# jacobhinkle/lagomorph

Measured on AMD Instinct MI355X. Metric: LDDMM step voxels/sec (3D, 128^3), higher is better.
Workload: dtype f32; 1 GPU; lddmm.expmap, 10 Euler steps, global batch 32 x 3x128^3 fp32 sharded 32 per GPU (BASELINE configs[3]); value counts voxels x Euler steps; shooting from the identity, the first Euler step is evaluated in closed form (-dt sharp(m0): the bits EPDiff_step returns); the product's default path: each rank's shoot runs as 2 sub-batches on HIP streams of their own (lddmm.EXPMAP_STREAMS, bit-identical); streams=2, global_batch=32, per_gpu_batch=32, euler_steps=10

## Files before the change

### lagomorph_amd/csrc/fused.hip

```cpp
#include <algorithm>
#include <type_traits>
#include <stdlib.h>

#include "common.hpp"
#include "stencil_tile.hpp"
#include "gather_window.hpp"

namespace lago {

template <typename R, int DIM>
__global__ __launch_bounds__(kBlock) void compose_kernel(R *__restrict__ out, const R *__restrict__ u,
                                                         const R *__restrict__ v, double ds, double dt, Geom g) {
    const Vox vx = locate(g);
    if (!vx.valid) return;
    const size_t nv = g.nvox;
    const R *un = u + (size_t)vx.n * DIM * nv + vx.s;
    const R *vn = v + (size_t)vx.n * DIM * nv;
    R *on = out + (size_t)vx.n * DIM * nv + vx.s;
    const R dsr = (R)ds, dtr = (R)dt;
    R uv[DIM];
#pragma unroll
    for (int d = 0; d < DIM; ++d) uv[d] = un[(size_t)d * nv];
    if (DIM == 3) {
        Lerp3<R> L;
// ... 78 lines not shown
    const int lz = threadIdx.x & 31, ly = (threadIdx.x >> 5) & (GW::TY - 1), lxb = threadIdx.x / (32 * GW::TY);
    const int j = tl.y0 + ly, k = tl.z0 + lz;

    GWOrigin o;
    {
        const int cxi = min(tl.x0 + GW::TX / 2, g.nx - 1), cyi = min(tl.y0 + GW::TY / 2, g.ny - 1),
                  czi = min(tl.z0 + GW::TZ / 2, g.nz - 1);
        const uint32_t cs = ((uint32_t)cxi * (uint32_t)g.ny + (uint32_t)cyi) * (uint32_t)g.nz + (uint32_t)czi;
        o = gw_origin(tl, g, lg_floor(sample_pos_t<float, UNIT>(cxi, ds, un[cs])),
                      lg_floor(sample_pos_t<float, UNIT>(cyi, ds, un[nv + cs])),
                      lg_floor(sample_pos_t<float, UNIT>(czi, ds, un[2 * nv + cs])));
    }
    GWLoader<NT> ld;
    ld.plan(o, g);
    ld.issue(vn, plane, gwin);

    const bool row_ok = j < g.ny && k < g.nz;
    const uint32_t off0 = (((uint32_t)(tl.x0 + lxb) * (uint32_t)g.ny + (uint32_t)j) * (uint32_t)g.nz + (uint32_t)k) * 4u;
    const uint32_t estep = (uint32_t)XS * (uint32_t)g.ny * (uint32_t)g.nz * 4u;
    auto voff = [&](int e) { return row_ok && tl.x0 + lxb + XS * e < g.nx ? off0 + (uint32_t)e * estep : GW::kOutside; };
    GWLerp L[U];
    uint32_t outm = 0;
    float uu[3][U];
    {
#pragma unroll
        for (int e = 0; e < U; ++e) {
#pragma unroll
            for (int d = 0; d < 3; ++d)
                uu[d][e] = __builtin_bit_cast(float, __builtin_amdgcn_raw_buffer_load_b32(make_rsrc(un + (size_t)d * nv, plane), voff(e), 0, LAGO_COMPOSE_AUX_LD));
        }
#pragma unroll
        for (int e = 0; e < U; ++e) {
            const int i = tl.x0 + lxb + XS * e;
            const bool in = L[e].setup(sample_pos_t<float, UNIT>(i, ds, uu[0][e]), sample_pos_t<float, UNIT>(j, ds, uu[1][e]),
                                       sample_pos_t<float, UNIT>(k, ds, uu[2][e]), g, o);
            outm |= (in | (voff(e) == GW::kOutside)) ? 0u : 1u << e;
            __builtin_amdgcn_sched_barrier(0);
        }
    }
    auto channels = [&](auto stray) {
        constexpr bool STRAY = decltype(stray)::value;
#pragma unroll
        for (int c = 0; c < 3; ++c) {
            if (c > 0) {
                asm volatile("s_waitcnt vmcnt(0)" ::: "memory");
                __syncthreads();
            }
            const BufRsrc ro = make_rsrc(on + (size_t)c * nv, plane);
#pragma unroll
            for (int e = 0; e < U; ++e) {
                float val = L[e].value(gwin);
                if constexpr (STRAY) {
                    const bool mine = outm & (1u << e);
                    if (__builtin_amdgcn_ballot_w64(mine) != 0) {
                        if (mine) {
                            const int i = tl.x0 + lxb + XS * e;
                            Lerp3<float, false> P;
                            P.setup(sample_pos_t<float, UNIT>(i, ds, uu[0][e]), sample_pos_t<float, UNIT>(j, ds, uu[1][e]),
                                    sample_pos_t<float, UNIT>(k, ds, uu[2][e]), g.nx, g.ny, g.nz);
                            val = P.value(vn + (size_t)c * nv);
                        }
                    }
                }
                const float a = dsr * uu[c][e];
                const float b = dtr * val;
                __builtin_amdgcn_raw_buffer_store_b32(__builtin_bit_cast(uint32_t, a + b), ro, voff(e), 0, LAGO_COMPOSE_AUX_ST);
            }
            if (c < 2) {
                __syncthreads();
                ld.issue(vn + (size_t)(c + 1) * nv, plane, gwin);
            }
        }
    };
    asm volatile("s_waitcnt vmcnt(0)" ::: "memory");
    if (__syncthreads_or(outm != 0))
        channels(std::true_type{});
    else
        channels(std::false_type{});
}

template __global__ void compose3_window_kernel<GW::NT, 8, true>(float *, const float *, const float *, double, double, Geom, GWGrid);
template __global__ void compose3_window_kernel<GW::NT, 8, false>(float *, const float *, const float *, double, double, Geom, GWGrid);

std::atomic<int> g_gather_window{1};
std::atomic<int> g_tile_cube{1};

static size_t padded_smem(size_t smem) {
#ifdef LAGO_PROFILING
    static const size_t pad = [] {
        const char *e = getenv("LAGO_EXP_GATHER_PAD");
        return e ? (size_t)strtoul(e, nullptr, 10) : (size_t)0;
    }();
    if (pad > smem) smem = pad;
#endif
    return smem;
}

template <typename R>
static int compose_window_launch(R *out, const R *u, const R *v, double ds, double dt, const Geom &g, int64_t nn,
                                 hipStream_t s) {
    if constexpr (sizeof(R) == 4) {
        GWGrid w;
        if (!make_gwgrid(w, g, nn) || ((uintptr_t)v & 15u)) return kNotTaken;
        constexpr int NT = GW::NT, U = 8;
        const hipError_t e = with_flags([&](auto UNIT) {
            return launch(compose3_window_kernel<NT, U, UNIT()>, dim3(w.total), dim3(NT), padded_smem(GW::lds_bytes<NT>()), s,
                          out, u, v, ds, dt, g, w);
        }, unit_dt<R>(ds));
        if (e != hipSuccess) return fail_hip(e, "compose");
        note_path(LP_GATHER_WINDOW);
        return LAGO_OK;
    }
    return kNotTaken;
}

template <typename R>
static int compose_impl(R *out, const R *u, const R *v, double ds, double dt, int dim, int64_t nn, int64_t nx,
                        int64_t ny, int64_t nz, void *stream) {
    if (dim != 2 && dim != 3) return fail_invalid("Only two- and three-dimensional interpolation is supported");
    Geom g;
    if (!make_geom(g, dim, nn, nx, ny, nz)) return fail_invalid("compose: bad extent");
    if (g.nblocks == 0) return LAGO_OK;
    if (!out || !u || !v) return fail_invalid("compose: null pointer");
    hipStream_t s = (hipStream_t)stream;
    constexpr int U = 2;
    if (dim == 3 && g_interp_vec && g_gather_window && g.nvox >= 32768u) {
        const int rc = compose_window_launch(out, u, v, ds, dt, g, nn, s);
        if (rc != kNotTaken) return rc != LAGO_OK ? rc : finish_launch(s, "compose");
    }
    uint32_t nbx_u, nb;
    if (dim == 3 && g_interp_vec && slab_grid(g, nn, U, nbx_u, nb)) {
        with_flags([&](auto UNIT) {
            hipLaunchKernelGGL((compose3_unroll_kernel<R, U, UNIT()>), dim3(nb), dim3(kBlock), 0, s, out, u, v, ds, dt, g,
                               nbx_u, nb);
        }, unit_dt<R>(ds));
        note_path(LP_VECTOR_GATHER);
        return finish_launch(s, "compose");
    }
    with_dim(dim, [&](auto DIM) {
        hipLaunchKernelGGL((compose_kernel<R, DIM()>), dim3(g.nblocks), dim3(kBlock), 0, s, out, u, v, ds, dt, g);
    });
    return finish_launch(s, "compose");
}


template <typename R, int DIM>
__device__ __forceinline__ R jac_row_dot(int c, const R (&fp)[DIM], const R (&fm)[DIM], const R (&w)[DIM]) {
    R gq[DIM];
#pragma unroll
    for (int d = 0; d < DIM; ++d) {
        gq[d] = (R)0.5f * (fp[d] - fm[d]);
        if (c == d) gq[d] = gq[d] + (R)1.0;
    }
    const R sacc = lg_fma(gq[0], w[0], gq[1] * w[1]);
    return DIM == 3 ? lg_fma(gq[DIM - 1], w[DIM - 1], sacc) : sacc;
}

template <typename R, int DIM>
__global__ __launch_bounds__(kBlock) void ad_star_kernel(R *__restrict__ out, R *__restrict__ mphi,
                                                         const R *__restrict__ phi, const R *__restrict__ m, Geom g) {
    const Vox vx = locate(g);
    if (!vx.valid) return;
    const size_t nv = g.nvox;
    const R *pn = phi + (size_t)vx.n * DIM * nv + vx.s;
    const R *mn = m + (size_t)vx.n * DIM * nv;
    R *on = out + (size_t)vx.n * DIM * nv + vx.s;
    R pv[DIM], wv[DIM];
#pragma unroll
    for (int d = 0; d < DIM; ++d) pv[d] = pn[(size_t)d * nv];
    int plus[DIM], minus[DIM];
    if (DIM == 3) {
        Lerp3<R> L;
        L.setup(sample_pos<R>(vx.i, 1.0, pv[0]), sample_pos<R>(vx.j, 1.0, pv[1]), sample_pos<R>(vx.k, 1.0, pv[2]),
                g.nx, g.ny, g.nz);
#pragma unroll
        for (int d = 0; d < 3; ++d) wv[d] = L.value(mn + (size_t)d * nv);
        const int P[3] = {vx.i, vx.j, vx.k}, Ln[3] = {g.nx, g.ny, g.nz}, St[3] = {g.ny * g.nz, g.nz, 1};
#pragma unroll
        for (int d = 0; d < 3; ++d) {
            plus[d] = P[d] + 1 < Ln[d] ? St[d] : 0;
            minus[d] = P[d] > 0 ? -St[d] : 0;
        }
    } else {
        Lerp2<R> L;
        L.setup(sample_pos<R>(vx.j, 1.0, pv[0]), sample_pos<R>(vx.k, 1.0, pv[1]), g.ny, g.nz);
#pragma unroll
// ... 202 lines not shown
template <typename R>
static int ad_star_impl(R *out, R *mphi, const R *phi, const R *m, int dim, int64_t nn, int64_t nx, int64_t ny,
                        int64_t nz, void *stream) {
    if (dim != 2 && dim != 3) return fail_invalid("Only two- and three-dimensional fields are supported");
    Geom g;
    if (!make_geom(g, dim, nn, nx, ny, nz)) return fail_invalid("ad_star: bad extent");
    if (g.nblocks == 0) return LAGO_OK;
    if (!out || !phi || !m) return fail_invalid("ad_star: null pointer");
    if (out == phi || out == m || (mphi && (mphi == phi || mphi == m || mphi == out)))
        return fail_invalid("ad_star: outputs may not alias an input or each other");
    if (thin(dim, nx, ny, nz))
        return fail_invalid("Jacobian times vectorfield not implemented for 'thin' dimensions");
    hipStream_t s = (hipStream_t)stream;
    constexpr int U = 2;
    if (dim == 3 && g_interp_vec && g_stencil_tile && g.nvox >= 4096u) {
        const int rc = ad_star_tile_launch<R>(out, mphi, phi, m, g, nn, s);
        if (rc != kNotTaken) return rc != LAGO_OK ? rc : finish_launch(s, "ad_star");
    }
    uint32_t nbx_u, nb;
    if (dim == 3 && g_interp_vec && slab_grid(g, nn, U, nbx_u, nb)) {
        hipLaunchKernelGGL((ad_star3_unroll_kernel<R, U>), dim3(nb), dim3(kBlock), 0, s, out, mphi, phi, m, g, nbx_u, nb);
        note_path(LP_VECTOR_GATHER);
        return finish_launch(s, "ad_star");
    }
    with_dim(dim, [&](auto DIM) {
        hipLaunchKernelGGL((ad_star_kernel<R, DIM()>), dim3(g.nblocks), dim3(kBlock), 0, s, out, mphi, phi, m, g);
    });
    return finish_launch(s, "ad_star");
}

template <typename R, int K, int VEC>
__global__ __launch_bounds__(256) void lincomb_kernel(R *out, const R *x0, const R *x1, const R *x2, const R *x3, R c0,
                                                      R c1, R c2, R c3, size_t nvec, int rev) {
    struct alignas(sizeof(R) * VEC) V { R e[VEC]; };
    const size_t stride = (size_t)gridDim.x * blockDim.x;
    for (size_t j = (size_t)blockIdx.x * blockDim.x + threadIdx.x; j < nvec; j += stride) {
        const size_t i = rev ? nvec - 1 - j : j;
        const V a = reinterpret_cast<const V *>(x0)[i];
        V b = a, c = a, d = a, r;
        if (K > 1) b = reinterpret_cast<const V *>(x1)[i];
        if (K > 2) c = reinterpret_cast<const V *>(x2)[i];
        if (K > 3) d = reinterpret_cast<const V *>(x3)[i];
#pragma unroll
        for (int e = 0; e < VEC; ++e) {
            R acc = c0 * a.e[e];
            if (K > 1) acc = lg_fma(c1, b.e[e], acc);
            if (K > 2) acc = lg_fma(c2, c.e[e], acc);
            if (K > 3) acc = lg_fma(c3, d.e[e], acc);
            r.e[e] = acc;
        }
        reinterpret_cast<V *>(out)[i] = r;
    }
}

template <typename R>
int lincomb_impl(R *out, int k, const R *x0, const R *x1, const R *x2, const R *x3, double c0, double c1, double c2,
                 double c3, int64_t n, void *stream) {
    if (k < 1 || k > 4 || n < 0) return fail_invalid("lincomb: 1 to 4 terms");
    if (n == 0) return LAGO_OK;
    hipStream_t s = (hipStream_t)stream;
    constexpr int VEC = 16 / sizeof(R);
    auto aligned = [](const void *p) { return p == nullptr || (reinterpret_cast<uintptr_t>(p) & 15) == 0; };
    const bool vec = n % VEC == 0 && aligned(out) && aligned(x0) && aligned(k > 1 ? x1 : nullptr) &&
                     aligned(k > 2 ? x2 : nullptr) && aligned(k > 3 ? x3 : nullptr);
    const size_t nvec = vec ? (size_t)n / VEC : (size_t)n;
    const uint32_t grid = (uint32_t)std::min<size_t>((nvec + 255) / 256, (size_t)256 * 32);
    const int rev = next_direction();
    with_flags([&](auto WIDE) {
        constexpr int V = WIDE() ? VEC : 1;
        with_int<1, 2, 3, 4>(k, [&](auto K) {
            hipLaunchKernelGGL((lincomb_kernel<R, K(), V>), dim3(grid), dim3(256), 0, s, out, x0, x1, x2, x3, (R)c0, (R)c1,
                               (R)c2, (R)c3, nvec, rev);
        });
    }, vec);
    return finish_launch(s, "lincomb");
}

}

namespace lago {
void tune_fused(int stencil_tile, int gather_window) {
    g_stencil_tile = stencil_tile ? 1 : 0;
    g_tile_cube = stencil_tile == 3 ? 0 : 1;
    g_gather_window = gather_window ? 1 : 0;
}
}

extern "C" {
int lago_lincomb_f32(float *out, int k, const float *x0, const float *x1, const float *x2, const float *x3, double c0,
                     double c1, double c2, double c3, int64_t n, void *stream) {
    return lago::lincomb_impl<float>(out, k, x0, x1, x2, x3, c0, c1, c2, c3, n, stream);
}
int lago_lincomb_f64(double *out, int k, const double *x0, const double *x1, const double *x2, const double *x3,
                     double c0, double c1, double c2, double c3, int64_t n, void *stream) {
    return lago::lincomb_impl<double>(out, k, x0, x1, x2, x3, c0, c1, c2, c3, n, stream);
}
int lago_compose_f32(float *out, const float *u, const float *v, double ds, double dt, int dim, int64_t nn,
                     int64_t nx, int64_t ny, int64_t nz, void *stream) {
    return lago::compose_impl<float>(out, u, v, ds, dt, dim, nn, nx, ny, nz, stream);
}
int lago_compose_f64(double *out, const double *u, const double *v, double ds, double dt, int dim, int64_t nn,
                     int64_t nx, int64_t ny, int64_t nz, void *stream) {
    return lago::compose_impl<double>(out, u, v, ds, dt, dim, nn, nx, ny, nz, stream);
}
int lago_Ad_star_f32(float *out, float *mphi, const float *phiinv, const float *m, int dim, int64_t nn, int64_t nx,
                     int64_t ny, int64_t nz, void *stream) {
    return lago::ad_star_impl<float>(out, mphi, phiinv, m, dim, nn, nx, ny, nz, stream);
}
int lago_Ad_star_f64(double *out, double *mphi, const double *phiinv, const double *m, int dim, int64_t nn, int64_t nx,
                     int64_t ny, int64_t nz, void *stream) {
    return lago::ad_star_impl<double>(out, mphi, phiinv, m, dim, nn, nx, ny, nz, stream);
}
}
```

### lagomorph_amd/csrc/gather_window.hpp

```cpp
#pragma once
#include "common.hpp"

namespace lago {

struct GW {
#ifndef LAGO_GW_TY
#define LAGO_GW_TY 16
#endif
    static constexpr int TX = 8, TY = LAGO_GW_TY, TZ = 32, H = 2, HZ = 4;
    static constexpr int NT = 32 * TY;
    static constexpr int WX = TX + 1 + 2 * H, WY = TY + 1 + 2 * H, WZC = 11, WZ = 4 * WZC;
    static constexpr int NCHUNK = WX * WY * WZC;
    static constexpr uint32_t kOutside = 0x80000000u;
    template <int NT>
    static constexpr int rounds() { return (NCHUNK + NT - 1) / NT; }
    template <int NT>
    static constexpr size_t lds_bytes() { return (size_t)rounds<NT>() * NT * 16; }
};

struct GWGrid {
    uint32_t ntx, nty, ntz, per_item, total;
    FastDiv d_item, d_tz, d_ty;
};

inline bool make_gwgrid(GWGrid &w, const Geom &g, int64_t nn) {
    if (g.nz < 4 || (g.nz & 3) || g.nx < 2 || g.ny < 2) return false;
    w.ntx = (g.nx + GW::TX - 1) / GW::TX;
    w.nty = (g.ny + GW::TY - 1) / GW::TY;
    w.ntz = (g.nz + GW::TZ - 1) / GW::TZ;
    w.per_item = w.ntx * w.nty * w.ntz;
    const uint64_t total = (uint64_t)w.per_item * (uint64_t)nn;
    if (total == 0 || total >= (1ull << 31)) return false;
    if ((double)g.nvox < 0.85 * (double)w.per_item * (GW::TX * GW::TY * GW::TZ)) return false;
    w.total = (uint32_t)total;
    w.d_item = FastDiv(w.per_item);
    w.d_tz = FastDiv(w.ntz);
    w.d_ty = FastDiv(w.nty);
    return true;
}

struct GWTile {
    uint32_t n;
    int x0, y0, z0;
};
__device__ __forceinline__ GWTile gw_tile(const GWGrid &w, int rev) {
    const uint32_t L = block_order(blockIdx.x, w.total, rev);
    GWTile t;
    t.n = w.d_item.div(L);
    const uint32_t tb = L - t.n * w.per_item;
    const uint32_t txy = w.d_tz.div(tb);
    const uint32_t tx = w.d_ty.div(txy);
    t.z0 = (int)(tb - txy * w.ntz) * GW::TZ;
    t.y0 = (int)(txy - tx * w.nty) * GW::TY;
    t.x0 = (int)tx * GW::TX;
    return t;
}

struct GWOrigin {
    int ox, oy, oz;
};
__device__ __forceinline__ GWOrigin gw_origin(const GWTile &t, const Geom &g, int px, int py, int pz) {
    const int cxi = min(t.x0 + GW::TX / 2, g.nx - 1), cyi = min(t.y0 + GW::TY / 2, g.ny - 1),
              czi = min(t.z0 + GW::TZ / 2, g.nz - 1);
    GWOrigin o;
    o.ox = t.x0 + (px - cxi) - GW::H;
    o.oy = t.y0 + (py - cyi) - GW::H;
    o.oz = (t.z0 + (pz - czi) - GW::HZ) & ~3;
    return o;
}

template <int NT>
struct GWLoader {
    uint32_t src[GW::rounds<NT>()];
    __device__ __forceinline__ void plan(const GWOrigin &o, const Geom &g) {
#pragma unroll
        for (int r = 0; r < GW::rounds<NT>(); ++r) {
            const uint32_t c = (uint32_t)(r * NT) + threadIdx.x;
            const uint32_t row = c / (uint32_t)GW::WZC, cz = c - row * GW::WZC;
            const uint32_t wx = row / (uint32_t)GW::WY, wy = row - wx * GW::WY;
            const int gx = o.ox + (int)wx, gy = o.oy + (int)wy, gz = o.oz + 4 * (int)cz;
            const bool ok = c < (uint32_t)GW::NCHUNK && (uint32_t)gx < (uint32_t)g.nx && (uint32_t)gy < (uint32_t)g.ny &&
                            (uint32_t)gz < (uint32_t)g.nz;
            src[r] = ok ? (((uint32_t)gx * (uint32_t)g.ny + (uint32_t)gy) * (uint32_t)g.nz + (uint32_t)gz) * 4u : GW::kOutside;
        }
    }
    __device__ __forceinline__ void issue(const float *__restrict__ plane, uint32_t plane_bytes, float *win) const {
        const BufRsrc r = make_rsrc(plane, plane_bytes);
#pragma unroll
        for (int q = 0; q < GW::rounds<NT>(); ++q) {
            float *dst = win + (size_t)(q * NT + (threadIdx.x & ~63u)) * 4;
            __builtin_amdgcn_raw_ptr_buffer_load_lds(r, (__attribute__((address_space(3))) void *)dst, 16, src[q], 0, 0, 0);
        }
    }
};

struct GWLerp {
    float t, u, v;
    uint32_t pk;
    __device__ __forceinline__ bool setup(float x, float y, float z, const Geom &g, const GWOrigin &o) {
        const int flx = lg_floor(x), fly = lg_floor(y), flz = lg_floor(z);
        t = x - (float)flx;
        u = y - (float)fly;
        v = z - (float)flz;
        const int fx = clamp1(flx, g.nx), cx = clamp1(flx + 1, g.nx);
        const int fy = clamp1(fly, g.ny), cy = clamp1(fly + 1, g.ny);
        const int fz = clamp1(flz, g.nz), cz = clamp1(flz + 1, g.nz);
        const int zb = min(fz, g.nz - 2);
        const bool f_hi = fz != zb, c_lo = cz == zb;
        const int ax = fx - o.ox, ay = fy - o.oy, az = zb - o.oz;
        const bool in = ((uint32_t)ax < (uint32_t)(GW::WX - (cx - fx))) & ((uint32_t)ay < (uint32_t)(GW::WY - (cy - fy))) &
                        ((uint32_t)az < (uint32_t)(GW::WZ - 1));
        const uint32_t wi = in ? (uint32_t)((ax * GW::WY + ay) * GW::WZ + az) : 0u;
        pk = wi | (cx != fx ? 1u << 14 : 0u) | (cy != fy ? 1u << 15 : 0u) | (f_hi ? 1u << 16 : 0u) | (c_lo ? 1u << 17 : 0u);
        asm volatile("" : "+v"(pk), "+v"(t), "+v"(u), "+v"(v));
        return in;
    }
    __device__ __forceinline__ float value(const float *win) const {
        uint32_t p = pk;
        asm volatile("" : "+v"(p));
        const uint32_t b0 = p & 0x3fffu;
        const uint32_t dX = (p & (1u << 14)) ? (uint32_t)(GW::WY * GW::WZ) : 0u, dY = (p & (1u << 15)) ? (uint32_t)GW::WZ : 0u;
        const bool f_hi = p & (1u << 16), c_lo = p & (1u << 17);
        const uint32_t rb[4] = {b0, b0 + dX, b0 + dX + dY, b0 + dY};
        float lo[4], hi[4];
#pragma unroll
        for (int q = 0; q < 4; ++q) { lo[q] = win[rb[q]]; hi[q] = win[rb[q] + 1]; }
        return lerp3_pairs(lo, hi, t, u, v, f_hi, c_lo);
    }
};

}
```

### lagomorph_amd/lagomorph_ext.py

```python
import ctypes
import math
import threading
import os

import torch

_HERE = os.path.dirname(os.path.abspath(__file__))
LIB_PATH = os.environ.get("LAGO_HIP_LIBRARY") or os.path.join(_HERE, "_lib", "liblagomorph_hip.so")
ABI_VERSION = 5

if not os.path.exists(LIB_PATH):
    raise ImportError(
        f"{LIB_PATH} not found: the HIP extension is not built "
        "(run `python -m lagomorph_amd.build`); lagomorph_amd has no CPU fallback"
    )
_lib = ctypes.CDLL(LIB_PATH)
_lib.lago_abi_version.restype = ctypes.c_int
if _lib.lago_abi_version() != ABI_VERSION:
    raise ImportError(
        f"{LIB_PATH} has C-ABI version {_lib.lago_abi_version()}, this binding needs {ABI_VERSION}: "
        "rebuild it with `python -m lagomorph_amd.build -f`"
    )
_lib.lago_last_error.restype = ctypes.c_char_p
_lib.lago_version.restype = ctypes.c_char_p
# ... 141 lines not shown
    d = t.dim() - 2
    if d == 2:
        return 2, t.size(2), t.size(3), 1
    if d == 3:
        return 3, t.size(2), t.size(3), t.size(4)
    return d, 0, 0, 0


def _call(name, ref, *args):
    f = _fn[name + _suffix(ref)]
    if ref.device.index != torch.cuda.current_device():
        with torch.cuda.device(ref.device):
            rc = f(*args, torch.cuda.current_stream().cuda_stream)
    else:
        rc = f(*args, torch.cuda.current_stream().cuda_stream)
    if rc != 0:
        raise RuntimeError(_lib.lago_last_error().decode("utf-8", "replace"))


def _ptr(t):
    return t.data_ptr() if t is not None and t.numel() > 0 else None




def set_debug_mode(mode):
    _lib.lago_set_debug(1 if mode else 0)


def set_splat_mode(mode):
    tune(splat_mode=mode)


def set_splat_tile(tx, ty, tz, mx, my, mz, nthreads):
    tune(splat_tile=[tx, ty, tz, mx, my, mz, nthreads])


def set_splat_shear(on=1, tx=8, ty=6, tz=0, mx=1, my=1, mz=4, nthreads=1024):
    tune(splat_shear=[on, tx, ty, tz, mx, my, mz, nthreads])


def set_splat_mc(on):
    tune(splat_mc=1 if on else 0)


def set_splat_shear_mc(mode):
    tune(splat_shear_mc=mode)


def set_fluid_tuning(xpass_ipw=0, zy_persist=1, xpass_wide=1, xpass_persist=1):
    tune(fluid_xpass_persist=xpass_persist, fluid_xpass_ipw=xpass_ipw, fluid_zy_persist=1 if zy_persist else 0,
         fluid_xpass_wide=1 if xpass_wide else 0)


def set_launch_order(alternate):
    tune(launch_order=1 if alternate else 0)


def set_stencil_tile(on):
    tune(stencil_tile=on)


_lib.lago_path_launches.restype = ctypes.c_longlong
_lib.lago_path_launches.argtypes = [_int]
PATHS = ("gather_window", "stencil_tile", "vector_gather", "splat_shear", "splat_shear_mc", "splat_tiled", "splat_global",
         "fluid_lds", "fluid_2d", "fluid_xpass", "fluid_rocfft", "splat_2d", "splat_affine_box", "fluid_generic")


_lib.lago_reversed_launches.restype = ctypes.c_longlong
_lib.lago_reversed_launches.argtypes = []


def reversed_launches():
    return int(_lib.lago_reversed_launches())


def path_launches(name=None):
    if name is not None:
        return int(_lib.lago_path_launches(PATHS.index(name)))
    return {p: int(_lib.lago_path_launches(i)) for i, p in enumerate(PATHS)}


def set_gather_window(on):
    tune(gather_window=1 if on else 0)


if os.environ.get("LAGO_GATHER_WINDOW") is not None:
    set_gather_window(os.environ["LAGO_GATHER_WINDOW"].strip().lower() not in ("", "0", "off", "false", "no"))


def set_vector_kernels(on):
    tune(vector_kernels=1 if on else 0)


def set_fluid_mode(mode):
    tune(fluid_mode=mode)


def version():
    return _lib.lago_version().decode()


def interp_forward(Iv, u, dt=1.0):
    _check_input(Iv, "Iv")
    _check_input(u, "u")
    _same(Iv, u)
    dim, nx, ny, nz = _spatial(Iv)
    if dim not in (2, 3):
        raise RuntimeError("Only two- and three-dimensional interpolation is supported")
    if u.dim() != Iv.dim() or u.size(1) != dim or tuple(u.shape[2:]) != tuple(Iv.shape[2:]):
        raise RuntimeError(f"interp_forward: displacement of shape {tuple(u.shape)} does not match image {tuple(Iv.shape)}")
    nn = max(u.size(0), Iv.size(0))
    bc = Iv.size(0) < nn
    if (bc and Iv.size(0) != 1) or u.size(0) != nn:
        raise RuntimeError("interp_forward: batch sizes of I and u are incompatible")
    out = torch.empty((nn, Iv.size(1)) + tuple(Iv.shape[2:]), dtype=Iv.dtype, device=Iv.device)
    _call("lago_interp_forward", Iv, _ptr(out), _ptr(Iv), _ptr(u), float(dt), dim, nn, Iv.size(1), nx, ny, nz, int(bc))
    return out


def interp_backward(grad_out, I, u, dt, need_I, need_u):
    _check_input(grad_out, "grad_out")
    _check_input(I, "I")
    _check_input(u, "u")
    _same(I, u, grad_out)
    dim, nx, ny, nz = _spatial(I)
    if dim not in (2, 3):
        raise RuntimeError("Only two- and three-dimensional interpolation is supported")
    nn = max(u.size(0), I.size(0))
    bc = I.size(0) < nn
    if (bc and I.size(0) != 1) or u.size(0) != nn:
        raise RuntimeError("interp_backward: batch sizes of I and u are incompatible")
    if (tuple(grad_out.shape) != (nn, I.size(1)) + tuple(I.shape[2:]) or u.dim() != I.dim() or u.size(1) != dim
            or tuple(u.shape[2:]) != tuple(I.shape[2:])):
        raise RuntimeError("interp_backward: grad_out / I / u shapes are inconsistent")
    d_I = torch.empty_like(I)
    d_u = torch.empty_like(u)
    _call("lago_interp_backward", I, _ptr(d_I), _ptr(d_u), _ptr(grad_out), _ptr(I), _ptr(u), float(dt), dim, nn,
          I.size(1), nx, ny, nz, int(bc), int(bool(need_I)), int(bool(need_u)))
    return [d_I, d_u]


def interp_hessian_diagonal_image(Iv, u, dt):
    _check_input(Iv, "Iv")
    _check_input(u, "u")
    _same(Iv, u)
    if Iv.dim() != 4 or u.dim() != 4 or u.size(1) != 2:
        raise RuntimeError("interp_hessian_diagonal_image is only implemented for two-dimensional images")
    nn = max(u.size(0), Iv.size(0))
    out = torch.empty_like(Iv)
    _call("lago_interp_hessian_diagonal_image", Iv, _ptr(out), _ptr(u), float(dt), Iv.size(0), nn, Iv.size(1),
          Iv.size(2), Iv.size(3))
    return out


def _check_jtv(g, v):
    for x, nm in ((g, "g"), (v, "v")):
        if not isinstance(x, torch.Tensor) or not x.is_cuda:
            raise RuntimeError(f"{nm} must be a CUDA tensor")
    _same(g, v)


def jacobian_times_vectorfield_forward(g, v, displacement, transpose):
    _check_jtv(g, v)
    g, v = g.contiguous(), v.contiguous()
    dim, nx, ny, nz = _spatial(g)
    if dim not in (2, 3):
# ... 618 lines not shown
```

Measured before the change: 31.97 billion voxels/s.

## Add persistent double-buffered pipelined gather-window compose kernel with larger tiles

Adds a persistent compose kernel launched on at most 256 workgroups, each looping over a contiguous range of tiles. It double-buffers the LDS window so the next velocity channel or tile is fetched while the current one is interpolated, and it prefetches the next tile's displacement. It also uses larger 16x16x32 tiles with 1024 threads and an XCD-aware work split. The aim is to hide global-to-LDS load latency and amortise launch and setup cost, at the price of a large LDS footprint (one workgroup per CU) and complex barrier and waitcnt bookkeeping.

```diff
diff --git a/lagomorph_amd/csrc/fused.hip b/lagomorph_amd/csrc/fused.hip
--- a/lagomorph_amd/csrc/fused.hip
+++ b/lagomorph_amd/csrc/fused.hip
@@ -184,6 +184,216 @@
 template __global__ void compose3_window_kernel<GW::NT, 8, true>(float *, const float *, const float *, double, double, Geom, GWGrid);
 template __global__ void compose3_window_kernel<GW::NT, 8, false>(float *, const float *, const float *, double, double, Geom, GWGrid);
 
+template <typename G, bool UNIT, bool PRE_U>
+__global__ __launch_bounds__(G::NT) __attribute__((amdgpu_waves_per_eu(4, 4))) void compose3_window_pipe_kernel(
+    float *__restrict__ out, const float *__restrict__ u, const float *__restrict__ v, double ds, double dt, Geom g, GWGrid w) {
+    constexpr int NT = G::NT, XS = NT / (32 * G::TY), U = G::TX / XS;
+    static_assert(XS * U == G::TX && NT % (32 * G::TY) == 0, "tile shape");
+    extern __shared__ float gwin[];
+    constexpr uint32_t kBuf = (uint32_t)(G::trimmed_bytes() / 4);
+    const uint32_t T = w.total, Lw = xcd_swizzle(blockIdx.x, gridDim.x);
+    uint32_t q0, q1, qstep;
+    if (gridDim.x % 8u == 0 && T >= gridDim.x) {
+        const uint32_t gx = gridDim.x / 8u, x = Lw / gx;
+        q0 = (uint32_t)((uint64_t)x * T / 8u) + (Lw - x * gx);
+        q1 = (uint32_t)((uint64_t)(x + 1) * T / 8u);
+        qstep = gx;
+    } else {
+        q0 = (uint32_t)((uint64_t)Lw * T / gridDim.x);
+        q1 = (uint32_t)((uint64_t)(Lw + 1) * T / gridDim.x);
+        qstep = 1;
+    }
+    if (q0 >= q1) return;
+    const size_t nv = g.nvox;
+    const uint32_t plane = g.nvox * 4u;
+    const float dsr = (float)ds, dtr = (float)dt;
+    const uint32_t estep = (uint32_t)XS * (uint32_t)g.ny * (uint32_t)g.nz * 4u;
+
+    struct Lane {
+        int lxb, j, k;
+    };
+    auto lane_of = [&](const GWTile &tl) {
+        uint32_t tid = threadIdx.x;
+        asm volatile("" : "+v"(tid));
+        Lane a;
+        a.lxb = tid / (32 * G::TY);
+        a.j = tl.y0 + (int)((tid >> 5) & (G::TY - 1));
+        a.k = tl.z0 + (int)(tid & 31);
+        return a;
+    };
+    struct Tile {
+        GWTile tl;
+        uint32_t off0;
+        uint32_t m;
+    };
+    auto tile_of = [&](const GWTile &tl) {
+        Tile t;
+        t.tl = tl;
+        const Lane a = lane_of(tl);
+        t.off0 = (((uint32_t)(tl.x0 + a.lxb) * (uint32_t)g.ny + (uint32_t)a.j) * (uint32_t)g.nz + (uint32_t)a.k) * 4u;
+        const int ne = a.j < g.ny && a.k < g.nz ? (g.nx - tl.x0 - a.lxb + XS - 1) / XS : 0;
+        t.m = (1u << min(ne, U)) - 1u;
+        return t;
+    };
+    auto tile_no = [&](uint32_t q) { return gw_tile_at<G>(w, g.rev ? T - 1u - q : q); };
+    auto voff = [&](const Tile &t, int e) { return t.m & (1u << e) ? t.off0 + (uint32_t)e * estep : G::kOutside; };
+    auto un_of = [&](const GWTile &tl) { return u + (size_t)tl.n * 3 * nv; };
+    auto vn_of = [&](const GWTile &tl) { return v + (size_t)tl.n * 3 * nv; };
+    auto on_of = [&](const GWTile &tl) { return out + (size_t)tl.n * 3 * nv; };
+    auto centre = [&](const GWTile &tl) {
+        const int cxi = min(tl.x0 + G::TX / 2, g.nx - 1), cyi = min(tl.y0 + G::TY / 2, g.ny - 1),
+                  czi = min(tl.z0 + G::TZ / 2, g.nz - 1);
+        return ((uint32_t)cxi * (uint32_t)g.ny + (uint32_t)cyi) * (uint32_t)g.nz + (uint32_t)czi;
+    };
+    auto origin = [&](const GWTile &tl, float cu0, float cu1, float cu2) {
+        const int cxi = min(tl.x0 + G::TX / 2, g.nx - 1), cyi = min(tl.y0 + G::TY / 2, g.ny - 1),
+                  czi = min(tl.z0 + G::TZ / 2, g.nz - 1);
+        return gw_origin<G>(tl, g, lg_floor(sample_pos_t<float, UNIT>(cxi, ds, cu0)),
+                            lg_floor(sample_pos_t<float, UNIT>(cyi, ds, cu1)), lg_floor(sample_pos_t<float, UNIT>(czi, ds, cu2)));
+    };
+
+    GWLoader<NT, G, true> ld;
+    GWLerpT<G> L[U];
+    float uu[3][U];
+    GWOrigin o;
+    auto load_u = [&](const Tile &t, int e, float (&dst)[3][U]) {
+        uint32_t off = voff(t, e);
+        asm volatile("" : "+v"(off));
+#pragma unroll
+        for (int d = 0; d < 3; ++d)
+            dst[d][e] = __builtin_bit_cast(float, __builtin_amdgcn_raw_buffer_load_b32(make_rsrc(un_of(t.tl) + (size_t)d * nv, plane), off, 0, LAGO_COMPOSE_AUX_LD));
+    };
+    auto setup = [&](Tile &t) {
+        const Lane a = lane_of(t.tl);
+        uint32_t outm = 0;
+#pragma unroll
+        for (int e = 0; e < U; ++e) {
+            const int i = t.tl.x0 + a.lxb + XS * e;
+            const bool in = L[e].setup(sample_pos_t<float, UNIT>(i, ds, uu[0][e]), sample_pos_t<float, UNIT>(a.j, ds, uu[1][e]),
+                                       sample_pos_t<float, UNIT>(a.k, ds, uu[2][e]), g, o);
+            outm |= (in | !(t.m & (1u << e))) ? 0u : 1u << e;
+            __builtin_amdgcn_sched_barrier(0);
+        }
+        if (__builtin_amdgcn_ballot_w64(outm != 0) != 0) {
+            const float *vn = vn_of(t.tl);
+            float *on = on_of(t.tl);
+#pragma unroll
+            for (int e = 0; e < U; ++e) {
+                const bool mine = outm & (1u << e);
+                if (__builtin_amdgcn_ballot_w64(mine) != 0) {
+                    if (mine) {
+                        const int i = t.tl.x0 + a.lxb + XS * e;
+                        Lerp3<float, false> P;
+                        P.setup(sample_pos_t<float, UNIT>(i, ds, uu[0][e]), sample_pos_t<float, UNIT>(a.j, ds, uu[1][e]),
+                                sample_pos_t<float, UNIT>(a.k, ds, uu[2][e]), g.nx, g.ny, g.nz);
+#pragma unroll
+                        for (int c = 0; c < 3; ++c) {
+                            const float val = P.value(vn + (size_t)c * nv);
+                            const float sa = dsr * uu[c][e];
+                            const float sb = dtr * val;
+                            __builtin_amdgcn_raw_buffer_store_b32(__builtin_bit_cast(uint32_t, sa + sb), make_rsrc(on + (size_t)c * nv, plane),
+                                                                  t.off0 + (uint32_t)e * estep, 0, LAGO_COMPOSE_AUX_ST);
+                        }
+                    }
+                }
+                __builtin_amdgcn_sched_barrier(0);
+            }
+            t.m &= ~outm;
+        }
+    };
+    auto lerp_stage = [&](auto cc, const Tile &t, const float *win, auto &&after) {
+        constexpr int c = decltype(cc)::value;
+        const BufRsrc ro = make_rsrc(on_of(t.tl) + (size_t)c * nv, plane);
+#pragma unroll
+        for (int e = 0; e < U; ++e) {
+            const float val = L[e].value(win);
+            const float a = dsr * uu[c][e];
+            const float b = dtr * val;
+            __builtin_amdgcn_raw_buffer_store_b32(__builtin_bit_cast(uint32_t, a + b), ro, voff(t, e), 0, LAGO_COMPOSE_AUX_ST);
+            after(e);
+        }
+    };
+    auto none = [](int) {};
+    auto plan = [&] {
+        uint32_t tid = threadIdx.x;
+        asm volatile("" : "+v"(tid));
+        ld.plan(o, g, tid);
+    };
+#define LAGO_GWP_STAGE_END(NEWER)                                   \
+    asm volatile("s_waitcnt vmcnt(%0)" ::"n"(NEWER) : "memory"); \
+    __builtin_amdgcn_s_barrier();                                  \
+    asm volatile("" ::: "memory")
+
+    Tile t = tile_of(tile_no(q0));
+    {
+        const uint32_t cs = centre(t.tl);
+        const float *un = un_of(t.tl);
+        o = origin(t.tl, un[cs], un[nv + cs], un[2 * nv + cs]);
+    }
+    plan();
+    ld.issue(vn_of(t.tl), plane, gwin);
+#pragma unroll
+    for (int e = 0; e < U; ++e) load_u(t, e, uu);
+    setup(t);
+    LAGO_GWP_STAGE_END(0);
+    uint32_t cur = 0;
+    for (uint32_t q = q0;; q += qstep) {
+        const bool more = q + qstep < q1;
+        float *const wa = gwin + cur, *const wb = gwin + (kBuf - cur);
+
+        ld.issue(vn_of(t.tl) + nv, plane, wb);
+        lerp_stage(std::integral_constant<int, 0>{}, t, wa, none);
+        LAGO_GWP_STAGE_END(U);
+
+        ld.issue(vn_of(t.tl) + 2 * nv, plane, wa);
+        const GWTile tln = more ? tile_no(q + qstep) : t.tl;
+        uint32_t c0, c1, c2;
+        {
+            const uint32_t cb = centre(tln) * 4u;
+            const float *un = un_of(tln);
+            const BufRsrc r0 = make_rsrc(un, plane), r1 = make_rsrc(un + nv, plane), r2 = make_rsrc(un + 2 * nv, plane);
+            asm volatile("buffer_load_dword %0, %1, %2, 0 offen" : "=v"(c0) : "v"(cb), "s"(r0) : "memory");
+            asm volatile("buffer_load_dword %0, %1, %2, 0 offen" : "=v"(c1) : "v"(cb), "s"(r1) : "memory");
+            asm volatile("buffer_load_dword %0, %1, %2, 0 offen" : "=v"(c2) : "v"(cb), "s"(r2) : "memory");
+        }
+        lerp_stage(std::integral_constant<int, 1>{}, t, wb, none);
+        asm volatile("s_waitcnt vmcnt(%3)" : "+v"(c0), "+v"(c1), "+v"(c2) : "n"(U) : "memory");
+        __builtin_amdgcn_s_barrier();
+        asm volatile("" ::: "memory");
+
+        o = origin(tln, __builtin_bit_cast(float, __builtin_amdgcn_readfirstlane(c0)),
+                   __builtin_bit_cast(float, __builtin_amdgcn_readfirstlane(c1)),
+                   __builtin_bit_cast(float, __builtin_amdgcn_readfirstlane(c2)));
+        if (more) {
+            plan();
+            ld.issue(vn_of(tln), plane, wb);
+        }
+        Tile tn = tile_of(tln);
+        auto next_u = [&](int e) {
+            if constexpr (PRE_U) load_u(tn, e, uu);
+        };
+        lerp_stage(std::integral_constant<int, 2>{}, t, wa, next_u);
+        LAGO_GWP_STAGE_END(PRE_U ? 4 * U : U);
+        if (!more) break;
+
+        t = tn;
+        if constexpr (!PRE_U) {
+#pragma unroll
+            for (int e = 0; e < U; ++e) load_u(t, e, uu);
+        }
+        setup(t);
+        cur = kBuf - cur;
+    }
+#undef LAGO_GWP_STAGE_END
+}
+
+#ifndef LAGO_COMPOSE_PRE_U
+#define LAGO_COMPOSE_PRE_U 1
+#endif
+constexpr bool kComposePreU = LAGO_COMPOSE_PRE_U;
+template __global__ void compose3_window_pipe_kernel<GWP, true, kComposePreU>(float *, const float *, const float *, double, double, Geom, GWGrid);
+template __global__ void compose3_window_pipe_kernel<GWP, false, kComposePreU>(float *, const float *, const float *, double, double, Geom, GWGrid);
+
 std::atomic<int> g_gather_window{1};
 std::atomic<int> g_tile_cube{1};
 
@@ -203,7 +413,19 @@
                                  hipStream_t s) {
     if constexpr (sizeof(R) == 4) {
         GWGrid w;
-        if (!make_gwgrid(w, g, nn) || ((uintptr_t)v & 15u)) return kNotTaken;
+        if ((uintptr_t)v & 15u) return kNotTaken;
+        if (g_gather_window == 1 && make_gwgrid<GWP>(w, g, nn)) {
+            static_assert(2 * GWP::trimmed_bytes() <= 160 * 1024 && 4 * GWP::trimmed_bytes() > 160 * 1024, "one workgroup per CU");
+            const uint32_t grid = std::min<uint32_t>(256u, w.total);
+            const hipError_t e = with_flags([&](auto UNIT) {
+                return launch(compose3_window_pipe_kernel<GWP, UNIT(), kComposePreU>, dim3(grid), dim3(GWP::NT),
+                              padded_smem(2 * GWP::trimmed_bytes()), s, out, u, v, ds, dt, g, w);
+            }, unit_dt<R>(ds));
+            if (e != hipSuccess) return fail_hip(e, "compose");
+            note_path(LP_GATHER_WINDOW);
+            return LAGO_OK;
+        }
+        if (!make_gwgrid(w, g, nn)) return kNotTaken;
         constexpr int NT = GW::NT, U = 8;
         const hipError_t e = with_flags([&](auto UNIT) {
             return launch(compose3_window_kernel<NT, U, UNIT()>, dim3(w.total), dim3(NT), padded_smem(GW::lds_bytes<NT>()), s,
@@ -572,7 +794,7 @@
 void tune_fused(int stencil_tile, int gather_window) {
     g_stencil_tile = stencil_tile ? 1 : 0;
     g_tile_cube = stencil_tile == 3 ? 0 : 1;
-    g_gather_window = gather_window ? 1 : 0;
+    g_gather_window = gather_window == 2 ? 2 : gather_window ? 1 : 0;
 }
 }
 
diff --git a/lagomorph_amd/csrc/gather_window.hpp b/lagomorph_amd/csrc/gather_window.hpp
--- a/lagomorph_amd/csrc/gather_window.hpp
+++ b/lagomorph_amd/csrc/gather_window.hpp
@@ -3,12 +3,13 @@
 
 namespace lago {
 
-struct GW {
 #ifndef LAGO_GW_TY
 #define LAGO_GW_TY 16
 #endif
-    static constexpr int TX = 8, TY = LAGO_GW_TY, TZ = 32, H = 2, HZ = 4;
-    static constexpr int NT = 32 * TY;
+template <int TX_, int TY_, int XS_>
+struct GWShape {
+    static constexpr int TX = TX_, TY = TY_, TZ = 32, H = 2, HZ = 4;
+    static constexpr int NT = 32 * TY * XS_;
     static constexpr int WX = TX + 1 + 2 * H, WY = TY + 1 + 2 * H, WZC = 11, WZ = 4 * WZC;
     static constexpr int NCHUNK = WX * WY * WZC;
     static constexpr uint32_t kOutside = 0x80000000u;
@@ -16,22 +17,28 @@
     static constexpr int rounds() { return (NCHUNK + NT - 1) / NT; }
     template <int NT>
     static constexpr size_t lds_bytes() { return (size_t)rounds<NT>() * NT * 16; }
+    static constexpr size_t trimmed_bytes() { return (size_t)((NCHUNK + 63) / 64) * 64 * 16; }
+    static constexpr int IDXB = WX * WY * WZ <= (1 << 14) ? 14 : 15;
+    static_assert(WX * WY * WZ <= (1 << IDXB), "window index");
 };
+using GW = GWShape<8, LAGO_GW_TY, 1>;
+using GWP = GWShape<16, 16, 2>;
 
 struct GWGrid {
     uint32_t ntx, nty, ntz, per_item, total;
     FastDiv d_item, d_tz, d_ty;
 };
 
+template <typename G = GW>
 inline bool make_gwgrid(GWGrid &w, const Geom &g, int64_t nn) {
     if (g.nz < 4 || (g.nz & 3) || g.nx < 2 || g.ny < 2) return false;
-    w.ntx = (g.nx + GW::TX - 1) / GW::TX;
-    w.nty = (g.ny + GW::TY - 1) / GW::TY;
-    w.ntz = (g.nz + GW::TZ - 1) / GW::TZ;
+    w.ntx = (g.nx + G::TX - 1) / G::TX;
+    w.nty = (g.ny + G::TY - 1) / G::TY;
+    w.ntz = (g.nz + G::TZ - 1) / G::TZ;
     w.per_item = w.ntx * w.nty * w.ntz;
     const uint64_t total = (uint64_t)w.per_item * (uint64_t)nn;
     if (total == 0 || total >= (1ull << 31)) return false;
-    if ((double)g.nvox < 0.85 * (double)w.per_item * (GW::TX * GW::TY * GW::TZ)) return false;
+    if ((double)g.nvox < 0.85 * (double)w.per_item * (G::TX * G::TY * G::TZ)) return false;
     w.total = (uint32_t)total;
     w.d_item = FastDiv(w.per_item);
     w.d_tz = FastDiv(w.ntz);
@@ -43,58 +50,66 @@
     uint32_t n;
     int x0, y0, z0;
 };
-__device__ __forceinline__ GWTile gw_tile(const GWGrid &w, int rev) {
-    const uint32_t L = block_order(blockIdx.x, w.total, rev);
+template <typename G = GW>
+__device__ __forceinline__ GWTile gw_tile_at(const GWGrid &w, uint32_t L) {
     GWTile t;
     t.n = w.d_item.div(L);
     const uint32_t tb = L - t.n * w.per_item;
     const uint32_t txy = w.d_tz.div(tb);
     const uint32_t tx = w.d_ty.div(txy);
-    t.z0 = (int)(tb - txy * w.ntz) * GW::TZ;
-    t.y0 = (int)(txy - tx * w.nty) * GW::TY;
-    t.x0 = (int)tx * GW::TX;
+    t.z0 = (int)(tb - txy * w.ntz) * G::TZ;
+    t.y0 = (int)(txy - tx * w.nty) * G::TY;
+    t.x0 = (int)tx * G::TX;
     return t;
+}
+__device__ __forceinline__ GWTile gw_tile(const GWGrid &w, int rev) {
+    return gw_tile_at<GW>(w, block_order(blockIdx.x, w.total, rev));
 }
 
 struct GWOrigin {
     int ox, oy, oz;
 };
+template <typename G = GW>
 __device__ __forceinline__ GWOrigin gw_origin(const GWTile &t, const Geom &g, int px, int py, int pz) {
-    const int cxi = min(t.x0 + GW::TX / 2, g.nx - 1), cyi = min(t.y0 + GW::TY / 2, g.ny - 1),
-              czi = min(t.z0 + GW::TZ / 2, g.nz - 1);
+    const int cxi = min(t.x0 + G::TX / 2, g.nx - 1), cyi = min(t.y0 + G::TY / 2, g.ny - 1),
+              czi = min(t.z0 + G::TZ / 2, g.nz - 1);
     GWOrigin o;
-    o.ox = t.x0 + (px - cxi) - GW::H;
-    o.oy = t.y0 + (py - cyi) - GW::H;
-    o.oz = (t.z0 + (pz - czi) - GW::HZ) & ~3;
+    o.ox = t.x0 + (px - cxi) - G::H;
+    o.oy = t.y0 + (py - cyi) - G::H;
+    o.oz = (t.z0 + (pz - czi) - G::HZ) & ~3;
     return o;
 }
 
-template <int NT>
+template <int NT, typename G = GW, bool TRIM = false>
 struct GWLoader {
-    uint32_t src[GW::rounds<NT>()];
-    __device__ __forceinline__ void plan(const GWOrigin &o, const Geom &g) {
+    static constexpr int R = G::template rounds<NT>();
+    uint32_t src[R];
+    __device__ __forceinline__ void plan(const GWOrigin &o, const Geom &g, uint32_t tid = threadIdx.x) {
 #pragma unroll
-        for (int r = 0; r < GW::rounds<NT>(); ++r) {
-            const uint32_t c = (uint32_t)(r * NT) + threadIdx.x;
-            const uint32_t row = c / (uint32_t)GW::WZC, cz = c - row * GW::WZC;
-            const uint32_t wx = row / (uint32_t)GW::WY, wy = row - wx * GW::WY;
+        for (int r = 0; r < R; ++r) {
+            const uint32_t c = (uint32_t)(r * NT) + tid;
+            const uint32_t row = c / (uint32_t)G::WZC, cz = c - row * G::WZC;
+            const uint32_t wx = row / (uint32_t)G::WY, wy = row - wx * G::WY;
             const int gx = o.ox + (int)wx, gy = o.oy + (int)wy, gz = o.oz + 4 * (int)cz;
-            const bool ok = c < (uint32_t)GW::NCHUNK && (uint32_t)gx < (uint32_t)g.nx && (uint32_t)gy < (uint32_t)g.ny &&
+            const bool ok = c < (uint32_t)G::NCHUNK && (uint32_t)gx < (uint32_t)g.nx && (uint32_t)gy < (uint32_t)g.ny &&
                             (uint32_t)gz < (uint32_t)g.nz;
-            src[r] = ok ? (((uint32_t)gx * (uint32_t)g.ny + (uint32_t)gy) * (uint32_t)g.nz + (uint32_t)gz) * 4u : GW::kOutside;
+            src[r] = ok ? (((uint32_t)gx * (uint32_t)g.ny + (uint32_t)gy) * (uint32_t)g.nz + (uint32_t)gz) * 4u : G::kOutside;
         }
     }
     __device__ __forceinline__ void issue(const float *__restrict__ plane, uint32_t plane_bytes, float *win) const {
         const BufRsrc r = make_rsrc(plane, plane_bytes);
 #pragma unroll
-        for (int q = 0; q < GW::rounds<NT>(); ++q) {
+        for (int q = 0; q < R; ++q) {
             float *dst = win + (size_t)(q * NT + (threadIdx.x & ~63u)) * 4;
+            if (TRIM && q == R - 1 && (uint32_t)(q * NT) + (threadIdx.x & ~63u) >= (uint32_t)G::NCHUNK) break;
             __builtin_amdgcn_raw_ptr_buffer_load_lds(r, (__attribute__((address_space(3))) void *)dst, 16, src[q], 0, 0, 0);
         }
     }
 };
 
-struct GWLerp {
+template <typename G>
+struct GWLerpT {
+    static constexpr int B = G::IDXB;
     float t, u, v;
     uint32_t pk;
     __device__ __forceinline__ bool setup(float x, float y, float z, const Geom &g, const GWOrigin &o) {
@@ -108,19 +123,19 @@
         const int zb = min(fz, g.nz - 2);
         const bool f_hi = fz != zb, c_lo = cz == zb;
         const int ax = fx - o.ox, ay = fy - o.oy, az = zb - o.oz;
-        const bool in = ((uint32_t)ax < (uint32_t)(GW::WX - (cx - fx))) & ((uint32_t)ay < (uint32_t)(GW::WY - (cy - fy))) &
-                        ((uint32_t)az < (uint32_t)(GW::WZ - 1));
-        const uint32_t wi = in ? (uint32_t)((ax * GW::WY + ay) * GW::WZ + az) : 0u;
-        pk = wi | (cx != fx ? 1u << 14 : 0u) | (cy != fy ? 1u << 15 : 0u) | (f_hi ? 1u << 16 : 0u) | (c_lo ? 1u << 17 : 0u);
+        const bool in = ((uint32_t)ax < (uint32_t)(G::WX - (cx - fx))) & ((uint32_t)ay < (uint32_t)(G::WY - (cy - fy))) &
+                        ((uint32_t)az < (uint32_t)(G::WZ - 1));
+        const uint32_t wi = in ? (uint32_t)((ax * G::WY + ay) * G::WZ + az) : 0u;
+        pk = wi | (cx != fx ? 1u << B : 0u) | (cy != fy ? 2u << B : 0u) | (f_hi ? 4u << B : 0u) | (c_lo ? 8u << B : 0u);
         asm volatile("" : "+v"(pk), "+v"(t), "+v"(u), "+v"(v));
         return in;
     }
     __device__ __forceinline__ float value(const float *win) const {
         uint32_t p = pk;
         asm volatile("" : "+v"(p));
-        const uint32_t b0 = p & 0x3fffu;
-        const uint32_t dX = (p & (1u << 14)) ? (uint32_t)(GW::WY * GW::WZ) : 0u, dY = (p & (1u << 15)) ? (uint32_t)GW::WZ : 0u;
-        const bool f_hi = p & (1u << 16), c_lo = p & (1u << 17);
+        const uint32_t b0 = p & ((1u << B) - 1u);
+        const uint32_t dX = (p & (1u << B)) ? (uint32_t)(G::WY * G::WZ) : 0u, dY = (p & (2u << B)) ? (uint32_t)G::WZ : 0u;
+        const bool f_hi = p & (4u << B), c_lo = p & (8u << B);
         const uint32_t rb[4] = {b0, b0 + dX, b0 + dX + dY, b0 + dY};
         float lo[4], hi[4];
 #pragma unroll
@@ -128,5 +143,6 @@
         return lerp3_pairs(lo, hi, t, u, v, f_hi, c_lo);
     }
 };
+using GWLerp = GWLerpT<GW>;
 
 }
diff --git a/lagomorph_amd/lagomorph_ext.py b/lagomorph_amd/lagomorph_ext.py
--- a/lagomorph_amd/lagomorph_ext.py
+++ b/lagomorph_amd/lagomorph_ext.py
@@ -247,7 +247,7 @@
 
 
 def set_gather_window(on):
-    tune(gather_window=1 if on else 0)
+    tune(gather_window=2 if on == 2 else 1 if on else 0)
 
 
 if os.environ.get("LAGO_GATHER_WINDOW") is not None:
```

Result: no change. 32.26 billion voxels/s, median of 6 (+0.9%).
